# arghyasur1991/Spark-TTS

Measured on AMD Instinct MI355X. Metric: audio samples/sec (whole node), Spark-TTS-0.5B greedy, higher is better.
Workload: dtype bf16 weights + KV, fp32 activations/accumulate (LLM); vocoder: fp32 operands split into 2 bf16 planes, 3 products on the bf16 matrix pipe, fp32 accumulate

## Files before the change

### include/sparkmi_debug.h

```cpp
#ifndef SPARKMI_DEBUG_H
#define SPARKMI_DEBUG_H

#include "sparkmi.h"

#ifdef __cplusplus
extern "C" {
#endif

int smi_llm_time_kernel(smi_llm* h, int kernel, int layer, int iters, float* ms_avg, void* stream);
int smi_llm_debug_stamps(smi_llm* h, int kernel, int layer, double* out);
int smi_llm_engine(smi_llm* h, int32_t* enabled, int32_t* info, char* why, int n);
int smi_llm_set_engine(smi_llm* h, int on);
int smi_llm_engine_plan(const smi_llm_cfg* cfg, int ncu, int32_t* stats);
int smi_llm_engine_stamps(smi_llm* h, double* out, int cap);
int smi_llm_debug_hidden(smi_llm* h, float* out_host, int n);
int smi_llm_debug_read(smi_llm* h, int what, void* out_host, size_t cap, size_t* got);

int smi_llm_debug_set_kv(smi_llm* h, int layer, int slot, int pos0, int n, const float* k_host, const float* v_host);
int smi_llm_debug_get_kv(smi_llm* h, int layer, int slot, int pos0, int n, float* k_host, float* v_host);
int smi_llm_debug_layer(smi_llm* h, int layer, int M, const int32_t* rows_host, const float* hidden_host, int stage);
int smi_llm_debug_raw_stamps(smi_llm* h, unsigned long long* out, int n);
int smi_llm_debug_sample(smi_llm* h, const float* logits_host, int n_rows, uint64_t seed, int use_bound, int32_t* tokens_out);
int smi_llm_debug_penalize(smi_llm* h, const float* logits_host, int n_rows, const uint16_t* hist_host, const smi_penalty_params* pens,
                           const int32_t* emitted_host, float* logits_out, int32_t* argmax_out);
int smi_llm_debug_logprob(smi_llm* h, const float* logits_host, int n_rows, const float* temperature_host, const int32_t* tokens_host,
                          float* lp_out);

#ifdef __cplusplus
}
#endif
#endif
```

### spark-tts_amd/csrc/smi_llm.hip

```cpp
#include "smi_common.h"
#include <stdio.h>
#include <string.h>
#include <cmath>
#include <map>
#include <mutex>
#include <vector>

namespace {

constexpr int kMaxRows = SMI_MAX_ROWS;
constexpr int kHeadDim = 64;

struct RowDesc {
  int32_t slot, pos, token, flags;
};

struct SampRec {
  int32_t mode;
  int32_t top_k;
  float inv_temp, top_p;
  unsigned long long seed;
  int32_t has_seed, pad;
};

// ... 77 lines not shown
  int ldsb;
  int lt_shift;
  const float* part_o;
  int n_oheads;
  const float* hres;
  const float* gam;
  float* h2out;
  const float* Yin;
  const unsigned char* pf2_base; int pf2_slice, pf2_nslices;
  int wperm;
  int kseg;
  float4* slab;
  int slab_mt;
  const int* tlist;
  const Ctl* ctl;
};
__device__ __forceinline__ int smi_wlane(int lane, int wperm) {
  return wperm ? ((lane & 12) << 2) + ((lane >> 4) << 2) + (lane & 3) : lane;
}
constexpr int kMaxOHeads = 16;

__device__ __forceinline__ uint4 smi_ldw(const uint4* q) {
#ifndef SMI_W_PLAIN
  typedef uint32_t u32x4_t __attribute__((ext_vector_type(4)));
  const u32x4_t v = __builtin_nontemporal_load((const u32x4_t*)q);
  return make_uint4(v.x, v.y, v.z, v.w);
#else
  return *q;
#endif
}
// ... 1374 lines not shown
  if (!allow_has(a, n + 1)) s.y = -INFINITY;
  if (!allow_has(a, n + 2)) s.z = -INFINITY;
  if (!allow_has(a, n + 3)) s.w = -INFINITY;
}
template <int HV, int RT = 0>
__global__ __launch_bounds__(256 * HV) void k_lm(GemmP p, int ngroups_arg, int m0_launch) {
  constexpr int NTB = 2, NW = 4, U = 8, MT = 1;
  constexpr size_t kHalfBytes = (size_t)NW * NTB * MT * 1024 + 32 * 4 + NTB * 32 * 8;
  extern __shared__ __attribute__((aligned(16))) unsigned char smem_all[];
  const int half = HV == 2 ? (int)threadIdx.x >> 8 : 0;
  unsigned char* smem = smem_all + half * kHalfBytes;
  const int tid = threadIdx.x & 255, lane = tid & 63, wave = tid >> 6;
  const int KT = p.KT, NT = p.NT;
  const int m0 = m0_launch + 16 * half;
  const int M = p.M - m0 < 16 ? (p.M - m0 > 0 ? p.M - m0 : 0) : 16;
  const int ntl = RT ? p.tlist[0] : 0;
  const int ngroups = RT ? (ntl + NTB - 1) / NTB : ngroups_arg;
  float4* red = (float4*)smem;
  float* rarr = (float*)(smem + (size_t)NW * NTB * MT * 1024);
  float* bestv = rarr + 32;
  int* besti = (int*)(bestv + NTB * 32);
  const int k8 = lane >> 4, em = lane & 15;
  const int mrow = em < M ? em : (M > 0 ? M - 1 : 0);
  const int xrow = m0 + mrow < p.M ? m0 + mrow : p.M - 1;
  bf16x8 bf[U][3];
#pragma unroll
  for (int u = 0; u < U; ++u) {
    int j = wave + u * NW;
    j = j < KT ? j : KT - 1;
#pragma unroll
    for (int s = 0; s < 3; ++s) bf[u][s] = *(const bf16x8*)(p.XS + xs_off(j, s, k8, xrow, p.M));
  }
  uint4 w[U][NTB];
  auto load_w = [&](int g) {
#pragma unroll
    for (int u = 0; u < U; ++u) {
      int j = wave + u * NW;
      j = j < KT ? j : KT - 1;
#pragma unroll
      for (int nb = 0; nb < NTB; ++nb) {
        int nt = g * NTB + nb;
        nt = RT ? lm_tile(p.tlist, nt) : (nt < NT ? nt : NT - 1);
        w[u][nb] = smi_ldw(&p.W[((size_t)nt * KT + j) * 64 + lane]);
      }
    }
  };
  int g = blockIdx.x;
  if (g < ngroups) load_w(g);
  for (int m = wave; m < M; m += NW) {
    float v = smi_ss_lane_sum(p.sspart + (size_t)(m0 + m) * p.npart, p.npart, lane);
    v = smi_wave_sum(v);
    if (lane == 0) rarr[m] = 1.0f / sqrtf(v / (float)(KT * 32) + p.eps);
  }
  for (int i = tid; i < NTB * 32; i += 256) { bestv[i] = -INFINITY; besti[i] = 0x7fffffff; }
  __syncthreads();
  const float rn = rarr[mrow];
  for (; g < ngroups; g += gridDim.x) {
    f32x4 acc[3][NTB];
#pragma unroll
    for (int c = 0; c < 3; ++c)
#pragma unroll
      for (int a = 0; a < NTB; ++a) acc[c][a] = (f32x4){0.f, 0.f, 0.f, 0.f};
#pragma unroll
    for (int u = 0; u < U; ++u) {
      if (wave + u * NW < KT) {
#pragma unroll
        for (int nb = 0; nb < NTB; ++nb) {
          const bf16x8 a = __builtin_bit_cast(bf16x8, w[u][nb]);
          acc[2][nb] = __builtin_amdgcn_mfma_f32_16x16x32_bf16(a, bf[u][2], acc[2][nb], 0, 0, 0);
          acc[1][nb] = __builtin_amdgcn_mfma_f32_16x16x32_bf16(a, bf[u][1], acc[1][nb], 0, 0, 0);
          acc[0][nb] = __builtin_amdgcn_mfma_f32_16x16x32_bf16(a, bf[u][0], acc[0][nb], 0, 0, 0);
        }
      }
    }
    const int gn = g + gridDim.x;
    if (gn < ngroups) load_w(gn);
#pragma unroll
    for (int nb = 0; nb < NTB; ++nb) {
      const f32x4 t = (acc[2][nb] + acc[1][nb]) + acc[0][nb];
      red[(wave * NTB + nb) * 64 + lane] = make_float4(t[0], t[1], t[2], t[3]);
    }
    __syncthreads();
    if (wave < NTB) {
      const int nb = wave, nt = RT ? (g * NTB + nb < ntl ? p.tlist[1 + g * NTB + nb] : NT) : g * NTB + nb;
      if (nt < NT) {
        float4 s = red[(0 * NTB + nb) * 64 + lane];
#pragma unroll
        for (int wv = 1; wv < NW; ++wv) {
          const float4 t = red[(wv * NTB + nb) * 64 + lane];
          s.x += t.x; s.y += t.y; s.z += t.z; s.w += t.w;
        }
        s.x *= rn; s.y *= rn; s.z *= rn; s.w *= rn;
        const int n = nt * 16 + 4 * (lane >> 4);
        const bool valid = em < M;
        if (RT && valid) lm_mask4(p.ctl, p.rows[m0 + em].slot, n, s);
        if (valid && p.Y) {
          float* y = p.Y + (size_t)(m0 + em) * p.V + n;
          if (n + 0 < p.V) y[0] = s.x;
          if (n + 1 < p.V) y[1] = s.y;
          if (n + 2 < p.V) y[2] = s.z;
          if (n + 3 < p.V) y[3] = s.w;
        }
        float bv = -INFINITY;
        int bi = 0x7fffffff;
        const float sv[4] = {s.x, s.y, s.z, s.w};
#pragma unroll
        for (int r = 0; r < 4; ++r)
          if (n + r < p.V && sv[r] > bv) { bv = sv[r]; bi = n + r; }
#pragma unroll
        for (int o = 16; o <= 32; o <<= 1) {
// ... 12 lines not shown
  }
  if (tid < M) {
    float bv = -INFINITY;
    int bi = 0x7fffffff;
#pragma unroll
    for (int nb = 0; nb < NTB; ++nb) {
      const float ov = bestv[nb * 32 + tid];
      const int oi = besti[nb * 32 + tid];
      if (ov > bv || (ov == bv && oi < bi)) { bv = ov; bi = oi; }
    }
    p.pval[(size_t)(m0 + tid) * gridDim.x + blockIdx.x] = bv;
    p.pidx[(size_t)(m0 + tid) * gridDim.x + blockIdx.x] = bi;
  }
}


template <int UW, int RT = 0>
__global__ __launch_bounds__(256) void k_lm32(GemmP p, int ngroups_arg, int m0) {
  constexpr int NTB = 2, NW = 4, U = UW;
  extern __shared__ __attribute__((aligned(16))) unsigned char smem[];
  const int tid = threadIdx.x, lane = tid & 63, wave = tid >> 6;
  const int KT = p.KT, NT = p.NT;
  const int ntl = RT ? p.tlist[0] : 0;
  const int ngroups = RT ? (ntl + NTB - 1) / NTB : ngroups_arg;
  const int M = p.M - m0 < 32 ? p.M - m0 : 32;
  float4* red = (float4*)smem;
  float* rarr = (float*)(smem + (size_t)NW * NTB * 2 * 1024);
  float* bestv = rarr + 32;
  int* besti = (int*)(bestv + NTB * 32);
  uint4* xl = (uint4*)(smem + (size_t)NW * NTB * 2 * 1024 + 32 * 4 + NTB * 32 * 8);
// ... 1509 lines not shown
  Ctl hctl; Ctl* ctl;
  int admit_seq;
  int session, identity_slots;
  std::vector<int> live_order;
  int attn_seg;
  float* apart; size_t apart_floats;
  int slot_busy[kMaxRows], slot_len[kMaxRows];
  int max_len, steps_launched;
  int do_sample, top_k; float temperature, top_p; unsigned long long seed;
  int slot_samp[kMaxRows];
  int slot_pen[kMaxRows];
  int slot_lp[kMaxRows];
  int slot_allow[kMaxRows];
  int lm_restrict;
  int* tlist;
  std::vector<int32_t> host_tlist;
  float* lp;
  float* lp_part; float2* lp_rowc;
  uint16_t* phist;
  int64_t* poll_dev; int64_t* poll_host;
  int32_t* pen_idx; size_t pen_idx_cap;
  std::vector<int32_t> host_pen_idx;
  float* logits; int* tok;
  float* cand_v; int* cand_i; unsigned int* cand_n;
  unsigned long long* stamps; int stamps_on;
  int max_steps;
  int tune[4];
  int graph_steps;
  int pf_inline;
  int pf_qkv_eighths;
// ... 87 lines not shown
bool lp_any(const smi_llm* L) {
  for (int sl = 0; sl < kMaxRows; ++sl)
    if (L->slot_lp[sl]) return true;
  return false;
}
bool allow_any(const smi_llm* L) {
  for (int sl = 0; sl < kMaxRows; ++sl)
    if (L->slot_allow[sl]) return true;
  return false;
}
bool lm_restricted(const smi_llm* L) {
  return L->lm_restrict && L->KTh <= 32 && !L->exact && allow_any(L);
}
bool logits_needed(const smi_llm* L) {
  return samp_any(L) || pen_any(L) || lp_any(L) || (allow_any(L) && !lm_restricted(L));
}
int allow_bits(const smi_llm* L) { return allow_any(L) ? (lm_restricted(L) ? 3 : 1) : 0; }
uint64_t graph_key(const smi_llm* L, int samp, int pen, int lp, int K) {
  return (uint64_t)L->B | ((uint64_t)L->attn_seg << 8) | ((uint64_t)(L->identity_slots ? 1 : 0) << 24) | ((uint64_t)samp << 25) |
         ((uint64_t)pen << 26) | ((uint64_t)lp << 27) | ((uint64_t)allow_bits(L) << 28) | ((uint64_t)K << 32);
}
void graphs_flush(smi_llm* L) {
  std::vector<hipStream_t> drained;
  for (auto& gl : L->graph_last) {
    bool seen = false;
    for (hipStream_t d : drained) seen |= d == gl.second;
    if (!seen) { (void)hipStreamSynchronize(gl.second); drained.push_back(gl.second); }
  }
  L->graph_last.clear();
  for (auto& kv : L->graph_cache) if (kv.second) (void)hipGraphExecDestroy(kv.second);
// ... 247 lines not shown
enum { PF_GROUPED = 1, PF_PGEMM = 2 };
constexpr int kPgSplitRows = 512;
constexpr int kPgSegO = 2, kPgSegD = 8;

int ensure_apart(smi_llm* L, size_t floats) {
  if (floats <= L->apart_floats) return SMI_OK;
  graphs_flush(L);
  if (L->apart) (void)hipFree(L->apart);
  L->apart = nullptr; L->apart_floats = 0;
  if (hipMalloc((void**)&L->apart, floats * 4) != hipSuccess) { smi_set_error("hipMalloc(attention partials, %zu floats) failed", floats); return SMI_ENOMEM; }
  L->apart_floats = floats;
  return SMI_OK;
}

int lm_blocks_for(const smi_llm* L, int M) {
  if (L->KTh > 32 || L->exact) return L->lm_cap;
  return M <= 16 ? L->lm_blocks : (L->lm_blocks < 256 ? L->lm_blocks : 256);
}

int pen_set_ids(int V, int nblk) { return ((V + nblk - 1) / nblk + 3) & ~3; }

LpP lp_params(const smi_llm* L, int M) {
  LpP lp;
  lp.logits = L->logits; lp.ctl = L->ctl; lp.rows = L->rows; lp.pval = L->pval; lp.nblk = lm_blocks_for(L, M);
  lp.V = L->cfg.vocab_size; lp.per = pen_set_ids(lp.V, kLpBlocks); lp.inv_temp = 1.0f / L->temperature; lp.hs = L->do_sample;
  lp.part = L->lp_part; lp.rowc = L->lp_rowc;
  return lp;
}

int segs_for(int ctx_bound) { return ctx_bound <= kAttnSeg ? 1 : (ctx_bound + kAttnSeg - 1) / kAttnSeg; }
// ... 219 lines not shown
        const size_t lds = (size_t)4 * 2 * 1024 + 32 * 4 + 2 * 32 * 8;
        const size_t lds32 = (size_t)4 * 2 * 2 * 1024 + 32 * 4 + 2 * 32 * 8 + (size_t)L->KTh * 12 * 16 * 16;
        if (M <= 16) {
          hipLaunchKernelGGL((k_lm<1, 1>), dim3(L->lm_blocks), dim3(256), lds, st, p, 0, 0);
          SMI_LAUNCH_CHECK();
          return SMI_OK;
        }
        for (int m0 = 0; m0 < M; m0 += 32) {
          if (!(L->tune2 & 8192) && lds32 <= 150 * 1024) {
            if (L->KTh <= 28) hipLaunchKernelGGL((k_lm32<7, 1>), dim3(lm_blocks_for(L, M)), dim3(256), lds32, st, p, 0, m0);
            else hipLaunchKernelGGL((k_lm32<8, 1>), dim3(lm_blocks_for(L, M)), dim3(256), lds32, st, p, 0, m0);
          } else
            hipLaunchKernelGGL((k_lm<2, 1>), dim3(lm_blocks_for(L, M)), dim3(512), 2 * lds, st, p, 0, m0);
          SMI_LAUNCH_CHECK();
        }
        return SMI_OK;
      }
      if (L->KTh <= 32) {
        const int ngroups = (L->NTlm + 1) / 2;
        const size_t lds = (size_t)4 * 2 * 1024 + 32 * 4 + 2 * 32 * 8;
        if (M <= 16) {
          hipLaunchKernelGGL(k_lm<1>, dim3(L->lm_blocks), dim3(256), lds, st, p, ngroups, 0);
          SMI_LAUNCH_CHECK();
        } else {
          const size_t lds32 = (size_t)4 * 2 * 2 * 1024 + 32 * 4 + 2 * 32 * 8 + (size_t)L->KTh * 12 * 16 * 16;
          for (int m0 = 0; m0 < M; m0 += 32) {
            if (!(L->tune2 & 8192) && lds32 <= 150 * 1024) {
              if (L->KTh <= 28) hipLaunchKernelGGL(k_lm32<7>, dim3(lm_blocks_for(L, M)), dim3(256), lds32, st, p, ngroups, m0);
              else hipLaunchKernelGGL(k_lm32<8>, dim3(lm_blocks_for(L, M)), dim3(256), lds32, st, p, ngroups, m0);
            } else
// ... 323 lines not shown
    L->pg_forced = common;
    for (int i = 0; i < 4; ++i) { const char* e = smi_env(names[i]); L->pg_forced |= e != nullptr; L->pg_min[i] = e ? atoi(e) : common ? L->pgemm_min_rows : dflt[i]; }
  }
  { const char* e = smi_env("SPARKMI_PG_SPLIT_ROWS"); L->pg_split_rows = e ? atoi(e) : kPgSplitRows; if (L->pg_split_rows > kPgSplitRows) L->pg_split_rows = kPgSplitRows; }
  { const char* e = smi_env("SPARKMI_PF_LONG"); L->pf_long = e ? atoi(e) : kMaxRows + 1; if (L->pf_long < kMaxRows + 1) L->pf_long = kMaxRows + 1; }
  { const char* e = smi_env("SPARKMI_GU1_ROWS"); L->gu1_rows = e ? atoi(e) : 32; }
  { const char* e = smi_env("SPARKMI_GU1_LO"); L->gu1_lo = e ? atoi(e) : 4; }
  L->wd_parts = cfg->wd_plain ? 0 : 1;
  L->exact = cfg->weights_exact;
  if (L->exact) L->fuse_o = 0;
  L->pf_tiles = nullptr; L->pf_tiles_cap = 0; L->pf_ntiles = 0;
  { const char* e = smi_env("SPARKMI_ATTN_PF2"); L->attn_pf2 = !(e && e[0] == '0'); }
  L->graph = nullptr; L->graph_B = 0; L->graph_seg = 1; L->graph_ident = 1; L->graph_samp = 0; L->graph_pen = 0; L->graph_lp = 0; L->graph_allow = 0; memset(L->slot_samp, 0, sizeof(L->slot_samp)); memset(L->slot_pen, 0, sizeof(L->slot_pen));
  memset(L->slot_lp, 0, sizeof(L->slot_lp)); L->lp = nullptr; L->lp_part = nullptr; L->lp_rowc = nullptr;
  memset(L->slot_allow, 0, sizeof(L->slot_allow)); L->lm_restrict = 0; L->tlist = nullptr;
  L->poll_dev = nullptr; L->poll_host = nullptr;
  L->phist = nullptr; L->pen_idx = nullptr; L->pen_idx_cap = 0; L->plan = nullptr; L->plan_cap = 0; L->B = 0; L->started = 0; L->ctl = nullptr; L->admit_seq = 0; memset(&L->hctl, 0, sizeof(L->hctl));
  L->session = 0; L->identity_slots = 1; L->attn_seg = 1; L->apart = nullptr; L->apart_floats = 0; memset(L->slot_busy, 0, sizeof(L->slot_busy)); memset(L->slot_len, 0, sizeof(L->slot_len));
  const size_t esz = cfg->kv_dtype ? 4 : 2;
  L->paged = cfg->kv_page_tokens > 0; L->pshift = 0; L->ppslot = 0; L->ptab = nullptr;
  memset(L->slot_pages, 0, sizeof(L->slot_pages)); memset(L->plen, 0, sizeof(L->plen));
  L->kv_layer_elems = (size_t)cfg->max_slots * cfg->num_kv_heads * cfg->max_positions * kHeadDim;
  if (L->paged) {
    while ((1 << L->pshift) < cfg->kv_page_tokens) ++L->pshift;
    L->ppslot = cfg->max_positions >> L->pshift;
    L->kv_layer_elems = (size_t)cfg->kv_pages * cfg->num_kv_heads * cfg->kv_page_tokens * kHeadDim;
    L->hptab.assign((size_t)cfg->max_slots * L->ppslot, 0);
    for (int pg = cfg->kv_pages - 1; pg >= 0; --pg) L->free_pages.push_back(pg);
    L->page_ref.assign((size_t)cfg->kv_pages, 0);
  }
// ... 31 lines not shown
  SMI_ALLOC(L->logits, (size_t)kMaxRows * cfg->vocab_size * 4);
  SMI_ALLOC(L->phist, (size_t)cfg->max_slots * cfg->vocab_size * 2);
  SMI_ALLOC(L->tok, kMaxRows * 4);
  SMI_ALLOC(L->cand_v, (size_t)kMaxRows * kCandCap * 4);
  SMI_ALLOC(L->cand_i, (size_t)kMaxRows * kCandCap * 4);
  SMI_ALLOC(L->cand_n, kMaxRows * 4);
  SMI_HIP(hipMemset(L->cand_n, 0, kMaxRows * 4));
  SMI_ALLOC(L->stamps, (size_t)4096 * 8 * 8);
  SMI_ALLOC(L->kcache, kvbytes);
  SMI_ALLOC(L->vcache, kvbytes);
  SMI_ALLOC(L->lp, (size_t)L->max_steps * kMaxRows * 4);
  SMI_ALLOC(L->lp_part, (size_t)kMaxRows * kLpBlocks * 4);
  SMI_ALLOC(L->lp_rowc, (size_t)kMaxRows * sizeof(float2));
  SMI_ALLOC(L->tlist, ((size_t)L->NTlm + 1) * 4);
  SMI_HIP(hipMemset(L->tlist, 0, ((size_t)L->NTlm + 1) * 4));
  SMI_ALLOC(L->poll_dev, (size_t)kMaxRows * (1 + (size_t)L->max_steps) * 8);
#undef SMI_ALLOC
  if (hipHostMalloc((void**)&L->poll_host, (size_t)kMaxRows * (1 + (size_t)L->max_steps) * 8, hipHostMallocDefault) != hipSuccess) {
    L->poll_host = nullptr;
    smi_set_error("hipHostMalloc(poll_host, %zu bytes) failed", (size_t)kMaxRows * (1 + (size_t)L->max_steps) * 8);
    smi_llm_destroy(L);
    return SMI_ENOMEM;
  }
  if (hipMemset(L->kcache, 0, kvbytes) != hipSuccess || hipMemset(L->vcache, 0, kvbytes) != hipSuccess ||
      hipMemset(L->h, 0, (size_t)kMaxRows * L->H * 4) != hipSuccess ||
      hipMemset(L->xs_h, 0, (size_t)kMaxRows * L->H * 6) != hipSuccess ||
      hipMemset(L->xs_attn, 0, (size_t)kMaxRows * L->Q * 6) != hipSuccess ||
      hipMemset(L->xs_act, 0, (size_t)kMaxRows * L->I * 6) != hipSuccess ||
      hipMemset(L->sspart, 0, (size_t)kMaxRows * L->NTh * 4 * 4) != hipSuccess ||
      hipMemset(L->qbuf, 0, (size_t)kMaxRows * L->Q * 4) != hipSuccess ||
// ... 19 lines not shown
      return SMI_EHIP;
    }
    for (size_t i = 0; i < lds_big_kernels().size() && !done[dev]; ++i)
      if (hipFuncSetAttribute(lds_big_kernels()[i], hipFuncAttributeMaxDynamicSharedMemorySize, kLdsBigBytes) != hipSuccess) {
        smi_set_error("smi_llm_create: hipFuncSetAttribute(MaxDynamicSharedMemorySize) failed: %s", hipGetErrorString(hipGetLastError()));
        smi_llm_destroy(L);
        return SMI_EHIP;
      }
    done[dev] = true;
  }
  if (hipEventCreate(&L->ev0) != hipSuccess || hipEventCreate(&L->ev1) != hipSuccess) {
    smi_set_error("hipEventCreate failed");
    smi_llm_destroy(L);
    return SMI_EHIP;
  }
#ifdef SMI_DIAG
  L->eng_on = 0;
  snprintf(L->eng.why, sizeof(L->eng.why), "off (opt-in: SPARKMI_ENGINE=1 or smi_llm_set_engine)");
  { const char* e = smi_env("SPARKMI_ENGINE");
    if (e && e[0] == '1') {
      const int rce = eng_create(L);
      if (rce) { smi_llm_destroy(L); return rce; }
      L->eng_on = L->eng.enabled;
    }
  }
#endif
  *out = L;
  return SMI_OK;
}

int smi_llm_destroy(smi_llm* L) {
  if (!L) return SMI_OK;
  graphs_flush(L);
  eng_destroy(L);
  void* ptrs[] = {L->h, L->qbuf, L->xs_h, L->xs_attn, L->xs_act, L->sspart, L->part_o, L->h2, L->dpart, L->fuse_cnt, L->rows, L->plan, L->pf_tiles, L->pval, L->pidx, L->hist,
                  L->count, L->finished, L->step, L->ctl, L->ptab, L->kcache, L->vcache, L->logits, L->tok, L->cand_v, L->cand_i, L->cand_n, L->stamps, L->bh, L->bq, L->bxs_h, L->bxs_attn, L->bxs_act, L->bss, L->pslab, L->apart,
                  L->phist, L->pen_idx, L->lp, L->lp_part, L->lp_rowc, L->tlist, L->poll_dev};
  for (void* q : ptrs)
    if (q) (void)hipFree(q);
  if (L->poll_host) (void)hipHostFree(L->poll_host);
  if (L->ev0) (void)hipEventDestroy(L->ev0);
  if (L->ev1) (void)hipEventDestroy(L->ev1);
  delete L;
  return SMI_OK;
}

int smi_llm_set_sampling(smi_llm* L, int do_sample, float temperature, int top_k, float top_p, uint64_t seed) {
  SMI_REQUIRE(L, "smi_llm_set_sampling: null handle");
  if (do_sample) {
    SMI_REQUIRE(temperature > 0.f, "smi_llm_set_sampling: temperature must be > 0");
    SMI_REQUIRE(top_k >= 1 && top_k <= kSampleCap, "smi_llm_set_sampling: top_k must be in 1..%d", kSampleCap);
    SMI_REQUIRE(top_p > 0.f && top_p <= 1.f, "smi_llm_set_sampling: top_p must be in (0, 1]");
// ... 991 lines not shown
    if ((rc = launch_one(L, kernel, layer % nl, L->rows, L->B, nullptr, st))) return rc;
    SMI_HIP(hipEventRecord(L->ev0, st));
    for (int i = 0; i < iters; ++i) {
      const int l = kernel >= KLM ? 0 : (layer + 1 + i) % nl;
      if ((rc = launch_one(L, kernel, l, L->rows, L->B, nullptr, st))) return rc;
    }
    SMI_HIP(hipEventRecord(L->ev1, st));
  }
  SMI_HIP(hipEventSynchronize(L->ev1));
  float ms = 0.f;
  SMI_HIP(hipEventElapsedTime(&ms, L->ev0, L->ev1));
  *ms_avg = ms / iters;
  return SMI_OK;
}

int smi_llm_engine(smi_llm* L, int32_t* enabled, int32_t* info, char* why, int n) {
  SMI_REQUIRE(L, "smi_llm_engine: null handle");
  if (enabled) *enabled = L->eng.enabled && L->eng_on;
  if (info) { info[0] = L->eng.ncu; info[1] = L->eng.maxlen; info[2] = L->eng.lds; info[3] = L->eng.enabled; }
  if (why && n > 0) { strncpy(why, L->eng.why, (size_t)n - 1); why[n - 1] = 0; }
  return SMI_OK;
}

int smi_llm_set_engine(smi_llm* L, int on) {
  SMI_REQUIRE(L, "smi_llm_set_engine: null handle");
  int v = on ? 1 : 0;
  if (v && !L->eng.enabled) {
    SMI_HIP(hipDeviceSynchronize());
    const int rce = eng_create(L);
    if (rce) return rce;
// ... 346 lines not shown
```

### spark-tts_amd/sparkmi/_lib.py

```python
from __future__ import annotations

import ctypes as C
import os
from pathlib import Path

_HERE = Path(__file__).resolve().parent
LIB_PATH = Path(os.environ["SPARKMI_LIB"]) if os.environ.get("SPARKMI_LIB") else _HERE / "libsparkmi.so"

SMI_MAX_ROWS = 64
SMI_MAX_EOS = 4
ABI_VERSION = 4


class SparkMIError(RuntimeError):
    pass


class LLMCfg(C.Structure):
    _fields_ = [(n, C.c_int32) for n in (
        "vocab_size", "hidden_size", "num_layers", "num_heads", "num_kv_heads", "head_dim",
        "intermediate_size", "max_slots", "max_positions", "kv_dtype", "use_graph")] + [("rms_eps", C.c_float),
                                                                                        ("kv_page_tokens", C.c_int32), ("kv_pages", C.c_int32), ("wd_plain", C.c_int32),
                                                                                        ("weights_exact", C.c_int32)]

# ... 121 lines not shown
    "smi_llm_debug_stamps": (_I, [_VP, _I, _I, _P(C.c_double)]),
    "smi_llm_engine": (_I, [_VP, _P(C.c_int32), _P(C.c_int32), C.c_char_p, _I]),
    "smi_llm_set_engine": (_I, [_VP, _I]),
    "smi_llm_engine_plan": (_I, [_P(LLMCfg), _I, _P(C.c_int32)]),
    "smi_llm_engine_stamps": (_I, [_VP, _P(C.c_double), _I]),
    "smi_llm_debug_hidden": (_I, [_VP, _P(C.c_float), _I]),
    "smi_llm_debug_read": (_I, [_VP, _I, _VP, _SZ, _P(_SZ)]),
    "smi_llm_debug_raw_stamps": (_I, [_VP, _P(C.c_uint64), _I]),
    "smi_llm_debug_sample": (_I, [_VP, _P(C.c_float), _I, C.c_uint64, _I, _P(C.c_int32)]),
    "smi_llm_debug_logprob": (_I, [_VP, _P(C.c_float), _I, _P(C.c_float), _P(C.c_int32), _P(C.c_float)]),
    "smi_llm_debug_penalize": (_I, [_VP, _P(C.c_float), _I, _P(C.c_uint16), _P(PenaltyParams), _P(C.c_int32), _P(C.c_float),
                                    _P(C.c_int32)]),
    "smi_llm_debug_set_kv": (_I, [_VP, _I, _I, _I, _I, _P(C.c_float), _P(C.c_float)]),
    "smi_llm_debug_get_kv": (_I, [_VP, _I, _I, _I, _I, _P(C.c_float), _P(C.c_float)]),
    "smi_llm_debug_layer": (_I, [_VP, _I, _I, _P(C.c_int32), _P(C.c_float), _I]),
}

DIAG_PATH = LIB_PATH.with_name("libsparkmi_diag.so")


class _Lib:

    def __init__(self, cdll: C.CDLL, path: Path, is_diag: bool):
        self._cdll, self.path, self.is_diag = cdll, path, is_diag

    def __getattr__(self, name):
        return getattr(self._cdll, name)

    def check(self, rc: int, what: str = "") -> None:
        if rc != 0:
# ... 53 lines not shown
```

### spark-tts_amd/sparkmi/llm.py

```python
from __future__ import annotations

import ctypes as C
import itertools
import json
import warnings
from pathlib import Path
from typing import Iterable, List, Mapping, Optional, Sequence, Union

import numpy as np
import torch

from . import _lib
from .arena import llm_cfg_struct, pack_llm_arena
from .config import LLMConfig


EosLike = Union[None, int, Iterable[int]]
SAMPLING_KEYS = ("do_sample", "temperature", "top_k", "top_p", "seed")
PENALTY_KEYS = ("repetition_penalty", "presence_penalty", "frequency_penalty", "min_new_tokens", "penalize_prompt")
PENALTY_NEUTRAL = dict(repetition_penalty=1.0, presence_penalty=0.0, frequency_penalty=0.0, min_new_tokens=0)
LOGPROB_KEYS = ("return_log_probs",)
ALLOW_KEY = "allowed_token_ids"


# ... 616 lines not shown
        self._lib.check(self._lib.smi_llm_engine(self._h, C.byref(on), info, why, 200), "smi_llm_engine")
        return {"enabled": bool(on.value), "built": bool(info[3]), "cus": int(info[0]), "images_per_wave": int(info[1]),
                "lds_bytes": int(info[2]), "why": why.value.decode(errors="replace")}

    def set_engine(self, on: bool) -> None:
        self._need_diag("set_engine")
        self._lib.check(self._lib.smi_llm_set_engine(self._h, 1 if on else 0), "smi_llm_set_engine")

    def engine_stamps(self) -> np.ndarray:
        self._need_diag("engine_stamps")
        n = 3 * self.cfg.num_hidden_layers * 16
        out = (C.c_double * n)()
        self._lib.check(self._lib.smi_llm_engine_stamps(self._h, out, n), "smi_llm_engine_stamps")
        return np.array(out, dtype=np.float64).reshape(3, self.cfg.num_hidden_layers, 16)

    def debug_hidden(self) -> np.ndarray:
        self._need_diag("debug_hidden")
        out = np.zeros(self.cfg.hidden_size, dtype=np.float32)
        self._lib.check(self._lib.smi_llm_debug_hidden(self._h, out.ctypes.data_as(C.POINTER(C.c_float)), out.size), "smi_llm_debug_hidden")
        return out

    def debug_read(self, what: int) -> np.ndarray:
        self._need_diag("debug_read")
        buf = np.zeros(1 << 22, dtype=np.uint8)
        got = C.c_size_t(0)
        self._lib.check(self._lib.smi_llm_debug_read(self._h, int(what), buf.ctypes.data_as(C.c_void_p), buf.size, C.byref(got)),
                   "smi_llm_debug_read")
        return buf[: got.value].copy()

    def debug_set_kv(self, layer: int, slot: int, k: np.ndarray, v: np.ndarray, pos0: int = 0) -> None:
# ... 127 lines not shown
```

Before: 566,900.

## Screen lm_head tiles with int8 bound pass before exact greedy argmax

Adds an int8-quantized copy of the lm_head weights, built once at create time. Each greedy step then runs a screening kernel that computes rigorous upper and lower bounds on every vocab tile's logits with int8 MFMA. The exact 3-plane bf16 lm_head kernel then evaluates only the tiles whose upper bound can reach the best lower bound. This aims to cut the weight bandwidth of the large vocab projection for greedy decoding when no logits are needed. The cost is an extra kernel and launch, extra memory for the quantized copy, and dependence on how tight the bounds are.

```diff
diff --git a/include/sparkmi_debug.h b/include/sparkmi_debug.h
--- a/include/sparkmi_debug.h
+++ b/include/sparkmi_debug.h
@@ -25,6 +25,7 @@
                            const int32_t* emitted_host, float* logits_out, int32_t* argmax_out);
 int smi_llm_debug_logprob(smi_llm* h, const float* logits_host, int n_rows, const float* temperature_host, const int32_t* tokens_host,
                           float* lp_out);
+int smi_llm_debug_lm_screen(smi_llm* h, int32_t* info, int32_t* list, int cap, int32_t* n);
 
 #ifdef __cplusplus
 }
diff --git a/spark-tts_amd/csrc/smi_llm.hip b/spark-tts_amd/csrc/smi_llm.hip
--- a/spark-tts_amd/csrc/smi_llm.hip
+++ b/spark-tts_amd/csrc/smi_llm.hip
@@ -115,6 +115,10 @@
   int slab_mt;
   const int* tlist;
   const Ctl* ctl;
+  const float* scr_ub;
+  const float* scr_lb;
+  int scr_ntq, scr_nlb;
+  int* scr_list;
 };
 __device__ __forceinline__ int smi_wlane(int lane, int wperm) {
   return wperm ? ((lane & 12) << 2) + ((lane >> 4) << 2) + (lane & 3) : lane;
@@ -1519,8 +1523,12 @@
   const int KT = p.KT, NT = p.NT;
   const int m0 = m0_launch + 16 * half;
   const int M = p.M - m0 < 16 ? (p.M - m0 > 0 ? p.M - m0 : 0) : 16;
-  const int ntl = RT ? p.tlist[0] : 0;
-  const int ngroups = RT ? (ntl + NTB - 1) / NTB : ngroups_arg;
+  static_assert(RT != 2 || HV == 1, "the screened form is the 16-row kernel");
+  int ntl = RT == 1 ? p.tlist[0] : 0;
+  int ngroups = RT == 1 ? (ntl + NTB - 1) / NTB : ngroups_arg;
+  float* scr_lbs = (float*)(smem_all + kHalfBytes);
+  int* scr_wcnt = (int*)(scr_lbs + 16);
+  int* llist = scr_wcnt + NW;
   float4* red = (float4*)smem;
   float* rarr = (float*)(smem + (size_t)NW * NTB * MT * 1024);
   float* bestv = rarr + 32;
@@ -1545,12 +1553,91 @@
 #pragma unroll
       for (int nb = 0; nb < NTB; ++nb) {
         int nt = g * NTB + nb;
-        nt = RT ? lm_tile(p.tlist, nt) : (nt < NT ? nt : NT - 1);
+        if constexpr (RT == 2) nt = llist[1 + (nt < ntl ? nt : ntl - 1)];
+        else nt = RT ? lm_tile(p.tlist, nt) : (nt < NT ? nt : NT - 1);
         w[u][nb] = smi_ldw(&p.W[((size_t)nt * KT + j) * 64 + lane]);
       }
     }
   };
-  int g = blockIdx.x;
+  if constexpr (RT == 2) {
+    const int Mall = p.M < 16 ? p.M : 16;
+    for (int m = wave; m < Mall; m += NW) {
+      float v = -INFINITY;
+      for (int i = lane; i < p.scr_nlb; i += 64) v = fmaxf(v, p.scr_lb[(size_t)m * p.scr_nlb + i]);
+#pragma unroll
+      for (int o = 32; o > 0; o >>= 1) v = fmaxf(v, __shfl_xor(v, o, 64));
+      if (lane == 0) scr_lbs[m] = v;
+    }
+    __syncthreads();
+    constexpr int JX = 16;
+    const int Q4 = p.scr_ntq >> 2, J = (Q4 + 4 * 64 - 1) / (4 * 64);
+    unsigned long long packed = 0ull;
+    for (int m = 0; m < Mall; ++m) {
+      float4 u[JX];
+#pragma unroll
+      for (int j = 0; j < JX; ++j) {
+        const int qd = (wave * J + j) * 64 + lane;
+        u[j] = make_float4(-INFINITY, -INFINITY, -INFINITY, -INFINITY);
+        if (j < J && qd < Q4) u[j] = *(const float4*)(p.scr_ub + (size_t)m * p.scr_ntq + 4 * qd);
+      }
+      const float lb = scr_lbs[m];
+#pragma unroll
+      for (int j = 0; j < JX; ++j) {
+        const unsigned long long k4 = (u[j].x >= lb ? 1u : 0u) | (u[j].y >= lb ? 2u : 0u) | (u[j].z >= lb ? 4u : 0u) | (u[j].w >= lb ? 8u : 0u);
+        packed |= k4 << (4 * j);
+      }
+    }
+#pragma unroll
+    for (int j = 0; j < JX; ++j) {
+      const int qd = (wave * J + j) * 64 + lane;
+#pragma unroll
+      for (int c = 0; c < 4; ++c)
+        if (j >= J || qd >= Q4 || 4 * qd + c >= NT) packed &= ~(1ull << (4 * j + c));
+    }
+    int cnt = __popcll(packed);
+#pragma unroll
+    for (int o = 32; o > 0; o >>= 1) cnt += __shfl_xor(cnt, o, 64);
+    if (lane == 0) scr_wcnt[wave] = cnt;
+    __syncthreads();
+    int base = 0, ntot = 0;
+#pragma unroll
+    for (int wv = 0; wv < NW; ++wv) { if (wv < wave) base += scr_wcnt[wv]; ntot += scr_wcnt[wv]; }
+    const int G = gridDim.x, bx = blockIdx.x;
+    const unsigned long long below = (1ull << lane) - 1ull;
+    for (int j = 0; j < J; ++j) {
+      const int qd = (wave * J + j) * 64 + lane;
+      const int msk = (int)(packed >> (4 * j)) & 15;
+      if (__ballot(msk != 0) == 0ull) continue;
+      int pre = 0, tot = 0;
+#pragma unroll
+      for (int c = 0; c < 4; ++c) {
+        const unsigned long long b = __ballot((msk >> c) & 1);
+        pre += __popcll(b & below);
+        tot += __popcll(b);
+      }
+      int o = base + pre;
+#pragma unroll
+      for (int c = 0; c < 4; ++c)
+        if ((msk >> c) & 1) {
+          const int cg = o >> 1;
+          if (cg % G == bx) llist[1 + (cg / G) * 2 + (o & 1)] = 4 * qd + c;
+          if (bx == 0) p.scr_list[1 + o] = 4 * qd + c;
+          ++o;
+        }
+      base += tot;
+    }
+    const int NG = (ntot + 1) >> 1;
+    ntl = 0;
+    if (bx < NG) {
+      ntl = 2 * ((NG - 1 - bx) / G + 1);
+      if ((ntot & 1) && (NG - 1) % G == bx) ntl -= 1;
+    }
+    ngroups = (ntl + NTB - 1) / NTB;
+    if (bx == 0 && tid == 0) p.scr_list[0] = ntot;
+    __syncthreads();
+  }
+  int g = RT == 2 ? 0 : blockIdx.x;
+  const int gstep = RT == 2 ? 1 : gridDim.x;
   if (g < ngroups) load_w(g);
   for (int m = wave; m < M; m += NW) {
     float v = smi_ss_lane_sum(p.sspart + (size_t)(m0 + m) * p.npart, p.npart, lane);
@@ -1560,7 +1647,7 @@
   for (int i = tid; i < NTB * 32; i += 256) { bestv[i] = -INFINITY; besti[i] = 0x7fffffff; }
   __syncthreads();
   const float rn = rarr[mrow];
-  for (; g < ngroups; g += gridDim.x) {
+  for (; g < ngroups; g += gstep) {
     f32x4 acc[3][NTB];
 #pragma unroll
     for (int c = 0; c < 3; ++c)
@@ -1578,7 +1665,7 @@
         }
       }
     }
-    const int gn = g + gridDim.x;
+    const int gn = g + gstep;
     if (gn < ngroups) load_w(gn);
 #pragma unroll
     for (int nb = 0; nb < NTB; ++nb) {
@@ -1587,7 +1674,9 @@
     }
     __syncthreads();
     if (wave < NTB) {
-      const int nb = wave, nt = RT ? (g * NTB + nb < ntl ? p.tlist[1 + g * NTB + nb] : NT) : g * NTB + nb;
+      const int nb = wave;
+      const int nt = RT == 2 ? (g * NTB + nb < ntl ? llist[1 + g * NTB + nb] : NT)
+                             : RT ? (g * NTB + nb < ntl ? p.tlist[1 + g * NTB + nb] : NT) : g * NTB + nb;
       if (nt < NT) {
         float4 s = red[(0 * NTB + nb) * 64 + lane];
 #pragma unroll
@@ -1598,7 +1687,7 @@
         s.x *= rn; s.y *= rn; s.z *= rn; s.w *= rn;
         const int n = nt * 16 + 4 * (lane >> 4);
         const bool valid = em < M;
-        if (RT && valid) lm_mask4(p.ctl, p.rows[m0 + em].slot, n, s);
+        if (RT == 1 && valid) lm_mask4(p.ctl, p.rows[m0 + em].slot, n, s);
         if (valid && p.Y) {
           float* y = p.Y + (size_t)(m0 + em) * p.V + n;
           if (n + 0 < p.V) y[0] = s.x;
@@ -1641,6 +1730,7 @@
   }
 }
 
+#include "smi_lm_screen.h"
 
 template <int UW, int RT = 0>
 __global__ __launch_bounds__(256) void k_lm32(GemmP p, int ngroups_arg, int m0) {
@@ -3180,6 +3270,9 @@
   int slot_allow[kMaxRows];
   int lm_restrict;
   int* tlist;
+  int scr_on, scr_kt8, scr_blocks, scr_xblocks, scr_ntq;
+  uint4* scr_q; float4* scr_meta; float *scr_ub, *scr_lb; int* scr_list;
+  float scr_build_ms;
   std::vector<int32_t> host_tlist;
   float* lp;
   float* lp_part; float2* lp_rowc;
@@ -3297,6 +3390,9 @@
 }
 bool logits_needed(const smi_llm* L) {
   return samp_any(L) || pen_any(L) || lp_any(L) || (allow_any(L) && !lm_restricted(L));
+}
+bool lm_screen(const smi_llm* L, int M) {
+  return L->scr_on && M <= 16 && !logits_needed(L) && !allow_any(L);
 }
 int allow_bits(const smi_llm* L) { return allow_any(L) ? (lm_restricted(L) ? 3 : 1) : 0; }
 uint64_t graph_key(const smi_llm* L, int samp, int pen, int lp, int K) {
@@ -3574,6 +3670,7 @@
 }
 
 int lm_blocks_for(const smi_llm* L, int M) {
+  if (lm_screen(L, M)) return L->scr_xblocks;
   if (L->KTh > 32 || L->exact) return L->lm_cap;
   return M <= 16 ? L->lm_blocks : (L->lm_blocks < 256 ? L->lm_blocks : 256);
 }
@@ -3823,6 +3920,22 @@
             hipLaunchKernelGGL((k_lm<2, 1>), dim3(lm_blocks_for(L, M)), dim3(512), 2 * lds, st, p, 0, m0);
           SMI_LAUNCH_CHECK();
         }
+        return SMI_OK;
+      }
+      if (!logits && lm_screen(L, M)) {
+        LmScrP sp;
+        sp.Q = L->scr_q; sp.meta = L->scr_meta; sp.NT = L->NTlm; sp.KT8 = L->scr_kt8; sp.KT = L->KTh; sp.M = M; sp.V = c.vocab_size;
+        sp.XS = L->xs_h; sp.sspart = L->sspart; sp.npart = L->NTh * 4; sp.eps = c.rms_eps;
+        sp.ub = L->scr_ub; sp.lb = L->scr_lb; sp.NTq = L->scr_ntq;
+        if (L->scr_kt8 <= 14) hipLaunchKernelGGL(k_lm_screen<14>, dim3(L->scr_blocks), dim3(256), 0, st, sp);
+        else hipLaunchKernelGGL(k_lm_screen<16>, dim3(L->scr_blocks), dim3(256), 0, st, sp);
+        SMI_LAUNCH_CHECK();
+        p.Y = nullptr;
+        p.scr_ub = L->scr_ub; p.scr_lb = L->scr_lb; p.scr_ntq = L->scr_ntq; p.scr_nlb = L->scr_blocks; p.scr_list = L->scr_list;
+        const int G = L->scr_xblocks, cap = 2 * (((L->NTlm + 1) / 2 + G - 1) / G);
+        const size_t lds = (size_t)4 * 2 * 1024 + 32 * 4 + 2 * 32 * 8 + 16 * 4 + 4 * 4 + ((size_t)cap + 1) * 4;
+        hipLaunchKernelGGL((k_lm<1, 2>), dim3(G), dim3(256), lds, st, p, 0, 0);
+        SMI_LAUNCH_CHECK();
         return SMI_OK;
       }
       if (L->KTh <= 32) {
@@ -4176,6 +4289,7 @@
   L->graph = nullptr; L->graph_B = 0; L->graph_seg = 1; L->graph_ident = 1; L->graph_samp = 0; L->graph_pen = 0; L->graph_lp = 0; L->graph_allow = 0; memset(L->slot_samp, 0, sizeof(L->slot_samp)); memset(L->slot_pen, 0, sizeof(L->slot_pen));
   memset(L->slot_lp, 0, sizeof(L->slot_lp)); L->lp = nullptr; L->lp_part = nullptr; L->lp_rowc = nullptr;
   memset(L->slot_allow, 0, sizeof(L->slot_allow)); L->lm_restrict = 0; L->tlist = nullptr;
+  L->scr_on = 0; L->scr_q = nullptr; L->scr_meta = nullptr; L->scr_ub = nullptr; L->scr_lb = nullptr; L->scr_list = nullptr; L->scr_build_ms = 0.f;
   L->poll_dev = nullptr; L->poll_host = nullptr;
   L->phist = nullptr; L->pen_idx = nullptr; L->pen_idx_cap = 0; L->plan = nullptr; L->plan_cap = 0; L->B = 0; L->started = 0; L->ctl = nullptr; L->admit_seq = 0; memset(&L->hctl, 0, sizeof(L->hctl));
   L->session = 0; L->identity_slots = 1; L->attn_seg = 1; L->apart = nullptr; L->apart_floats = 0; memset(L->slot_busy, 0, sizeof(L->slot_busy)); memset(L->slot_len, 0, sizeof(L->slot_len));
@@ -4237,6 +4351,23 @@
   SMI_ALLOC(L->lp_rowc, (size_t)kMaxRows * sizeof(float2));
   SMI_ALLOC(L->tlist, ((size_t)L->NTlm + 1) * 4);
   SMI_HIP(hipMemset(L->tlist, 0, ((size_t)L->NTlm + 1) * 4));
+#ifndef SMI_NO_LM_SCREEN
+  { const char* e = smi_env("SPARKMI_LM_SCREEN"); L->scr_on = !L->exact && L->KTh <= 32 && L->NTlm <= 16384 && !(e && e[0] == '0'); }
+#endif
+  if (L->scr_on) {
+    L->scr_kt8 = (L->KTh + 1) / 2;
+    L->scr_blocks = (L->NTlm + 3) / 4 < 512 ? (L->NTlm + 3) / 4 : 512;
+    L->scr_xblocks = L->lm_blocks < 64 ? L->lm_blocks : 64;
+    L->scr_ntq = (L->NTlm + 3) & ~3;
+    SMI_ALLOC(L->scr_q, (size_t)L->NTlm * L->scr_kt8 * 1024);
+    SMI_ALLOC(L->scr_meta, (size_t)L->NTlm * 16 * sizeof(float4));
+    SMI_ALLOC(L->scr_ub, (size_t)16 * L->scr_ntq * 4);
+    SMI_ALLOC(L->scr_lb, (size_t)16 * L->scr_blocks * 4);
+    SMI_ALLOC(L->scr_list, ((size_t)L->NTlm + 1) * 4);
+    SMI_HIP(hipMemset(L->scr_ub, 0, (size_t)16 * L->scr_ntq * 4));
+    SMI_HIP(hipMemset(L->scr_lb, 0, (size_t)16 * L->scr_blocks * 4));
+    SMI_HIP(hipMemset(L->scr_list, 0, ((size_t)L->NTlm + 1) * 4));
+  }
   SMI_ALLOC(L->poll_dev, (size_t)kMaxRows * (1 + (size_t)L->max_steps) * 8);
 #undef SMI_ALLOC
   if (hipHostMalloc((void**)&L->poll_host, (size_t)kMaxRows * (1 + (size_t)L->max_steps) * 8, hipHostMallocDefault) != hipSuccess) {
@@ -4286,6 +4417,18 @@
     smi_llm_destroy(L);
     return SMI_EHIP;
   }
+  if (L->scr_on) {
+    bool ok = hipEventRecord(L->ev0, 0) == hipSuccess;
+    hipLaunchKernelGGL(k_lm_screen_build, dim3((L->NTlm + 3) / 4), dim3(256), 0, 0, (const uint4*)sec(L, SMI_LLM_LM_HEAD, 0), L->NTlm, L->KTh,
+                       L->scr_kt8, L->scr_q, L->scr_meta);
+    ok = ok && hipGetLastError() == hipSuccess && hipEventRecord(L->ev1, 0) == hipSuccess && hipDeviceSynchronize() == hipSuccess &&
+         hipEventElapsedTime(&L->scr_build_ms, L->ev0, L->ev1) == hipSuccess;
+    if (!ok) {
+      smi_set_error("smi_llm_create: building the lm_head screening copy failed: %s", hipGetErrorString(hipGetLastError()));
+      smi_llm_destroy(L);
+      return SMI_EHIP;
+    }
+  }
 #ifdef SMI_DIAG
   L->eng_on = 0;
   snprintf(L->eng.why, sizeof(L->eng.why), "off (opt-in: SPARKMI_ENGINE=1 or smi_llm_set_engine)");
@@ -4307,7 +4450,8 @@
   eng_destroy(L);
   void* ptrs[] = {L->h, L->qbuf, L->xs_h, L->xs_attn, L->xs_act, L->sspart, L->part_o, L->h2, L->dpart, L->fuse_cnt, L->rows, L->plan, L->pf_tiles, L->pval, L->pidx, L->hist,
                   L->count, L->finished, L->step, L->ctl, L->ptab, L->kcache, L->vcache, L->logits, L->tok, L->cand_v, L->cand_i, L->cand_n, L->stamps, L->bh, L->bq, L->bxs_h, L->bxs_attn, L->bxs_act, L->bss, L->pslab, L->apart,
-                  L->phist, L->pen_idx, L->lp, L->lp_part, L->lp_rowc, L->tlist, L->poll_dev};
+                  L->phist, L->pen_idx, L->lp, L->lp_part, L->lp_rowc, L->tlist, L->poll_dev,
+                  L->scr_q, L->scr_meta, L->scr_ub, L->scr_lb, L->scr_list};
   for (void* q : ptrs)
     if (q) (void)hipFree(q);
   if (L->poll_host) (void)hipHostFree(L->poll_host);
@@ -5329,6 +5473,20 @@
   return SMI_OK;
 }
 
+int smi_llm_debug_lm_screen(smi_llm* L, int32_t* info, int32_t* list, int cap, int32_t* n) {
+  SMI_REQUIRE(L, "smi_llm_debug_lm_screen: null handle");
+  if (info) { info[0] = L->scr_on; info[1] = L->scr_on ? L->scr_xblocks : 0; info[2] = L->NTlm; info[3] = (int32_t)(L->scr_build_ms * 1e3f); }
+  if (n) *n = 0;
+  if (!L->scr_on) return SMI_OK;
+  SMI_HIP(hipDeviceSynchronize());
+  int32_t cnt = 0;
+  SMI_HIP(hipMemcpy(&cnt, L->scr_list, 4, hipMemcpyDeviceToHost));
+  SMI_REQUIRE(cnt >= 0 && cnt <= L->NTlm, "smi_llm_debug_lm_screen: candidate count %d outside 0..%d", cnt, L->NTlm);
+  if (n) *n = cnt;
+  if (list && cap > 0 && cnt > 0) SMI_HIP(hipMemcpy(list, L->scr_list + 1, (size_t)(cnt < cap ? cnt : cap) * 4, hipMemcpyDeviceToHost));
+  return SMI_OK;
+}
+
 int smi_llm_engine(smi_llm* L, int32_t* enabled, int32_t* info, char* why, int n) {
   SMI_REQUIRE(L, "smi_llm_engine: null handle");
   if (enabled) *enabled = L->eng.enabled && L->eng_on;
diff --git a/spark-tts_amd/csrc/smi_lm_screen.h b/spark-tts_amd/csrc/smi_lm_screen.h
--- /dev/null
+++ b/spark-tts_amd/csrc/smi_lm_screen.h
@@ -0,0 +1,190 @@
+constexpr float kScrC = 8.0f;
+struct LmScrP {
+  const uint4* Q;
+  const float4* meta;
+  int NT, KT8, KT, M, V;
+  const unsigned char* XS;
+  const float* sspart; int npart; float eps;
+  float* ub;
+  float* lb;
+  int NTq;
+};
+
+__global__ __launch_bounds__(256) void k_lm_screen_build(const uint4* W, int NT, int KT, int KT8, uint4* Q, float4* meta) {
+  const int lane = threadIdx.x & 63, wave = threadIdx.x >> 6;
+  const int nt = blockIdx.x * 4 + wave;
+  if (nt >= NT) return;
+  const int kb = lane >> 4, r = lane & 15;
+  auto piece = [&](int u, int h, float* v) {
+    const int kt = 2 * u + (kb >> 1);
+    uint4 q = make_uint4(0, 0, 0, 0);
+    if (kt < KT) q = W[((size_t)nt * KT + kt) * 64 + ((kb & 1) * 2 + h) * 16 + r];
+    const uint32_t d[4] = {q.x, q.y, q.z, q.w};
+#pragma unroll
+    for (int e = 0; e < 4; ++e) { v[2 * e] = smi_bf16_to_f32(d[e] & 0xffffu); v[2 * e + 1] = smi_bf16_to_f32(d[e] >> 16); }
+  };
+  float a = 0.f;
+  for (int u = 0; u < KT8; ++u)
+#pragma unroll
+    for (int h = 0; h < 2; ++h) {
+      float v[8];
+      piece(u, h, v);
+#pragma unroll
+      for (int e = 0; e < 8; ++e) a = fmaxf(a, fabsf(v[e]));
+    }
+  a = fmaxf(a, __shfl_xor(a, 16, 64));
+  a = fmaxf(a, __shfl_xor(a, 32, 64));
+  const float s = a > 1e-30f ? a / 127.0f : 1.0f;
+  double err = 0.0;
+  int n1 = 0;
+  for (int u = 0; u < KT8; ++u) {
+    uint32_t out[4] = {0u, 0u, 0u, 0u};
+#pragma unroll
+    for (int h = 0; h < 2; ++h) {
+      float v[8];
+      piece(u, h, v);
+#pragma unroll
+      for (int e = 0; e < 8; ++e) {
+        int q = (int)rintf(v[e] / s);
+        q = q > 127 ? 127 : (q < -127 ? -127 : q);
+        err = fmax(err, fabs((double)v[e] - (double)s * (double)q));
+        n1 += q < 0 ? -q : q;
+        out[(h * 8 + e) >> 2] |= (uint32_t)(q & 255) << (8 * ((h * 8 + e) & 3));
+      }
+    }
+    Q[((size_t)nt * KT8 + u) * 64 + lane] = make_uint4(out[0], out[1], out[2], out[3]);
+  }
+  err = fmax(err, __shfl_xor(err, 16, 64));
+  err = fmax(err, __shfl_xor(err, 32, 64));
+  n1 += __shfl_xor(n1, 16, 64);
+  n1 += __shfl_xor(n1, 32, 64);
+  auto up32 = [](double d) -> float {
+    float f = (float)d;
+    if ((double)f < d) f = f > 0.f ? __uint_as_float(__float_as_uint(f) + 1u) : 1.17549435e-38f;
+    return f;
+  };
+  if (kb == 0) meta[(size_t)nt * 16 + r] = make_float4(s, up32(err), a, up32((double)s * (double)n1));
+}
+
+template <int UK>
+__global__ __launch_bounds__(256, 2) void k_lm_screen(LmScrP p) {
+  typedef int i32x4_t __attribute__((ext_vector_type(4)));
+  __shared__ float rarr[16];
+  __shared__ float lbw[4][16];
+  __shared__ float4 xstat[16];
+  __shared__ uint4 planes[2][16][64];
+  const int tid = threadIdx.x, lane = tid & 63, wave = tid >> 6;
+  const int kb = lane >> 4, em = lane & 15;
+  const int M = p.M, NT = p.NT, KT8 = p.KT8;
+  const int mrow = em < M ? em : M - 1;
+  const int stride = 4 * (int)gridDim.x;
+  int nt = (int)blockIdx.x * 4 + wave;
+  uint4 w[UK];
+  float4 mt[4];
+  auto load_w = [&](int t) {
+#pragma unroll
+    for (int u = 0; u < UK; ++u) w[u] = smi_ldw(&p.Q[((size_t)t * KT8 + (u < KT8 ? u : KT8 - 1)) * 64 + lane]);
+#pragma unroll
+    for (int r = 0; r < 4; ++r) mt[r] = p.meta[(size_t)t * 16 + 4 * kb + r];
+  };
+  if (nt < NT) load_w(nt);
+  for (int m = wave; m < M; m += 4) {
+    float v = smi_ss_lane_sum(p.sspart + (size_t)m * p.npart, p.npart, lane);
+    v = smi_wave_sum(v);
+    if (lane == 0) rarr[m] = 1.0f / sqrtf(v / (float)(p.KT * 32) + p.eps);
+  }
+  auto xpiece = [&](int m, int kt, int k8, float* x) {
+    uint4 t[3];
+#pragma unroll
+    for (int s = 0; s < 3; ++s) {
+      t[s] = make_uint4(0, 0, 0, 0);
+      if (kt < p.KT) t[s] = *(const uint4*)(p.XS + xs_off(kt, s, k8, m, M));
+    }
+    const uint32_t d[3][4] = {{t[0].x, t[0].y, t[0].z, t[0].w}, {t[1].x, t[1].y, t[1].z, t[1].w}, {t[2].x, t[2].y, t[2].z, t[2].w}};
+#pragma unroll
+    for (int e = 0; e < 4; ++e) {
+      x[2 * e] = (smi_bf16_to_f32(d[0][e] & 0xffffu) + smi_bf16_to_f32(d[1][e] & 0xffffu)) + smi_bf16_to_f32(d[2][e] & 0xffffu);
+      x[2 * e + 1] = (smi_bf16_to_f32(d[0][e] >> 16) + smi_bf16_to_f32(d[1][e] >> 16)) + smi_bf16_to_f32(d[2][e] >> 16);
+    }
+  };
+  for (int m = wave; m < M; m += 4) {
+    float x1 = 0.f, mx = 0.f;
+    for (int j = lane; j < p.KT * 4; j += 64) {
+      float x[8];
+      xpiece(m, j >> 2, j & 3, x);
+#pragma unroll
+      for (int e = 0; e < 8; ++e) { x1 += fabsf(x[e]); mx = fmaxf(mx, fabsf(x[e])); }
+    }
+#pragma unroll
+    for (int o = 32; o > 0; o >>= 1) { x1 += __shfl_xor(x1, o, 64); mx = fmaxf(mx, __shfl_xor(mx, o, 64)); }
+    const bool tinyx = !(mx >= 1e-30f);
+    const float vq0 = tinyx ? 0.f : 32000.0f / mx;
+    const float tq0 = tinyx ? 0.f : 1.0f / vq0;
+    if (lane == 0) xstat[m] = make_float4(x1 * (1.0f + 0x1p-13f), vq0, tq0, tinyx ? mx : 0.51f * tq0);
+  }
+  __syncthreads();
+  for (int i = tid; i < M * KT8 * 4; i += 256) {
+    const int m = i % M, kq = (i / M) & 3, u = i / (4 * M);
+    const float vq0 = xstat[m].y;
+    uint32_t oh[4] = {0u, 0u, 0u, 0u}, ol[4] = {0u, 0u, 0u, 0u};
+#pragma unroll
+    for (int h = 0; h < 2; ++h) {
+      float x[8];
+      xpiece(m, 2 * u + (kq >> 1), (kq & 1) * 2 + h, x);
+#pragma unroll
+      for (int e = 0; e < 8; ++e) {
+        const int pq = (int)rintf(x[e] * vq0);
+        const int plo = ((pq + 128) & 255) - 128;
+        const int phi = (pq - plo) >> 8;
+        oh[(h * 8 + e) >> 2] |= (uint32_t)(phi & 255) << (8 * ((h * 8 + e) & 3));
+        ol[(h * 8 + e) >> 2] |= (uint32_t)(plo & 255) << (8 * ((h * 8 + e) & 3));
+      }
+    }
+    planes[0][u][kq * 16 + m] = make_uint4(oh[0], oh[1], oh[2], oh[3]);
+    planes[1][u][kq * 16 + m] = make_uint4(ol[0], ol[1], ol[2], ol[3]);
+  }
+  __syncthreads();
+  const float4 xs4 = xstat[mrow];
+  const float X1 = xs4.x, tq = xs4.z, rho = xs4.w;
+  i32x4_t bh[UK], bl[UK];
+#pragma unroll
+  for (int u = 0; u < UK; ++u) {
+    const uint4 vh = planes[0][u < KT8 ? u : 0][kb * 16 + mrow], vl = planes[1][u < KT8 ? u : 0][kb * 16 + mrow];
+    bh[u] = (i32x4_t){(int)vh.x, (int)vh.y, (int)vh.z, (int)vh.w};
+    bl[u] = (i32x4_t){(int)vl.x, (int)vl.y, (int)vl.z, (int)vl.w};
+  }
+  const float rn = rarr[mrow];
+  const float cK = kScrC * (float)(p.KT * 32) * 0x1p-24f;
+  float lbest = -INFINITY;
+  for (; nt < NT; nt += stride) {
+    i32x4_t ah = (i32x4_t){0, 0, 0, 0}, al = (i32x4_t){0, 0, 0, 0};
+#pragma unroll
+    for (int u = 0; u < UK; ++u) {
+      if (u < KT8) {
+        const i32x4_t a = __builtin_bit_cast(i32x4_t, w[u]);
+        ah = __builtin_amdgcn_mfma_i32_16x16x64_i8(a, bh[u], ah, 0, 0, 0);
+        al = __builtin_amdgcn_mfma_i32_16x16x64_i8(a, bl[u], al, 0, 0, 0);
+      }
+    }
+    const float4 m4[4] = {mt[0], mt[1], mt[2], mt[3]};
+    const int nn = nt + stride;
+    if (nn < NT) load_w(nn);
+    float tu = -INFINITY;
+#pragma unroll
+    for (int r = 0; r < 4; ++r) {
+      const float Sf = 256.0f * (float)ah[r] + (float)al[r];
+      const float A = m4[r].x * (tq * Sf);
+      const float E = ((X1 * (m4[r].y + cK * m4[r].z) + rho * m4[r].w) + 0x1p-100f) * (1.0f + 0x1p-19f);
+      const float up = rn * (A + E), lo = rn * (A - E);
+      if (nt * 16 + 4 * kb + r < p.V) { tu = fmaxf(tu, up); lbest = fmaxf(lbest, lo); }
+    }
+    tu = fmaxf(tu, __shfl_xor(tu, 16, 64));
+    tu = fmaxf(tu, __shfl_xor(tu, 32, 64));
+    if (lane < 16 && em < M) p.ub[(size_t)em * p.NTq + nt] = tu;
+  }
+  lbest = fmaxf(lbest, __shfl_xor(lbest, 16, 64));
+  lbest = fmaxf(lbest, __shfl_xor(lbest, 32, 64));
+  if (lane < 16) lbw[wave][em] = lbest;
+  __syncthreads();
+  if (tid < M) p.lb[(size_t)tid * gridDim.x + blockIdx.x] = fmaxf(fmaxf(lbw[0][tid], lbw[1][tid]), fmaxf(lbw[2][tid], lbw[3][tid]));
+}
diff --git a/spark-tts_amd/sparkmi/_lib.py b/spark-tts_amd/sparkmi/_lib.py
--- a/spark-tts_amd/sparkmi/_lib.py
+++ b/spark-tts_amd/sparkmi/_lib.py
@@ -159,6 +159,7 @@
     "smi_llm_debug_set_kv": (_I, [_VP, _I, _I, _I, _I, _P(C.c_float), _P(C.c_float)]),
     "smi_llm_debug_get_kv": (_I, [_VP, _I, _I, _I, _I, _P(C.c_float), _P(C.c_float)]),
     "smi_llm_debug_layer": (_I, [_VP, _I, _I, _P(C.c_int32), _P(C.c_float), _I]),
+    "smi_llm_debug_lm_screen": (_I, [_VP, _P(C.c_int32), _P(C.c_int32), _I, _P(C.c_int32)]),
 }
 
 DIAG_PATH = LIB_PATH.with_name("libsparkmi_diag.so")
diff --git a/spark-tts_amd/sparkmi/llm.py b/spark-tts_amd/sparkmi/llm.py
--- a/spark-tts_amd/sparkmi/llm.py
+++ b/spark-tts_amd/sparkmi/llm.py
@@ -654,6 +654,17 @@
         self._lib.check(self._lib.smi_llm_engine_stamps(self._h, out, n), "smi_llm_engine_stamps")
         return np.array(out, dtype=np.float64).reshape(3, self.cfg.num_hidden_layers, 16)
 
+    def debug_lm_screen(self) -> dict:
+        self._need_diag("debug_lm_screen")
+        info = (C.c_int32 * 4)()
+        n = C.c_int32(0)
+        self._lib.check(self._lib.smi_llm_debug_lm_screen(self._h, info, None, 0, C.byref(n)), "smi_llm_debug_lm_screen")
+        tiles = np.zeros(max(int(n.value), 1), dtype=np.int32)
+        self._lib.check(self._lib.smi_llm_debug_lm_screen(self._h, info, tiles.ctypes.data_as(C.POINTER(C.c_int32)), tiles.size,
+                                                          C.byref(n)), "smi_llm_debug_lm_screen")
+        return dict(on=bool(info[0]), exact_blocks=int(info[1]), vocab_tiles=int(info[2]), build_us=int(info[3]),
+                    tiles=tiles[: int(n.value)].tolist())
+
     def debug_hidden(self) -> np.ndarray:
         self._need_diag("debug_hidden")
         out = np.zeros(self.cfg.hidden_size, dtype=np.float32)
```

Result: no change. 567,000, median of 2 (+0.0%).
